# Enigmatisms/AdaPT

Measured on AMD Instinct MI355X. Metric: Msamples/s (W*H*spp/s), unidirectional MIS path tracing, higher is better.
Workload: dtype f32

## Files before the change

### adapt_amd/csrc/rng.hpp

```cpp
#pragma once
#include "vec.hpp"
#include <stdint.h>

struct Philox {
    uint32_t key0, key1, ctr0;
    uint32_t draw;
    uint32_t blk;
    uint32_t nblk;
    uint32_t c[4], n[4];
};

APT_HD void philox4x32_10(uint32_t c0, uint32_t c1, uint32_t c2, uint32_t c3, uint32_t k0, uint32_t k1, uint32_t out[4]) {
#if defined(__HIP_DEVICE_COMPILE__)
    asm volatile("" : "+v"(k0));
#endif
#pragma unroll
    for (int r = 0; r < 10; r++) {
        uint64_t p0 = (uint64_t)0xD2511F53u * c0;
        uint64_t p1 = (uint64_t)0xCD9E8D57u * c2;
        uint32_t n0 = (uint32_t)(p1 >> 32) ^ c1 ^ k0;
        uint32_t n1 = (uint32_t)p1;
        uint32_t n2 = (uint32_t)(p0 >> 32) ^ c3 ^ k1;
        uint32_t n3 = (uint32_t)p0;
        c0 = n0; c1 = n1; c2 = n2; c3 = n3;
        k0 += 0x9E3779B9u; k1 += 0xBB67AE85u;
    }
    out[0] = c0; out[1] = c1; out[2] = c2; out[3] = c3;
}

APT_HD void rng_init(Philox& r, uint32_t pixel, uint32_t seed, uint32_t sample, uint32_t draw) {
    r.key0 = pixel; r.key1 = seed; r.ctr0 = sample; r.draw = draw; r.blk = 0xffffffffu; r.nblk = 0xffffffffu;
    r.c[0] = r.c[1] = r.c[2] = r.c[3] = 0u;
    r.n[0] = r.n[1] = r.n[2] = r.n[3] = 0u;
}
APT_HD uint32_t rng_u32(Philox& r) {
    const uint32_t d = r.draw++;
    const uint32_t b = d >> 2;
    const bool step = b != r.blk;
    if (step && b != r.nblk) { philox4x32_10(r.ctr0, b, 0u, 0u, r.key0, r.key1, r.n); r.nblk = b; }
    if (step) { r.c[0] = r.n[0]; r.c[1] = r.n[1]; r.c[2] = r.n[2]; r.c[3] = r.n[3]; r.blk = b; r.nblk = 0xffffffffu; }
    const uint32_t w = d & 3u, c0 = r.c[0], c1 = r.c[1], c2 = r.c[2], c3 = r.c[3];
    return (w == 0u) ? c0 : ((w == 1u) ? c1 : ((w == 2u) ? c2 : c3));
}
APT_HD void rng_open(Philox& r) {
    const uint32_t b = r.draw >> 2;
    philox4x32_10(r.ctr0, b, 0u, 0u, r.key0, r.key1, r.c); r.blk = b;
    philox4x32_10(r.ctr0, b + 1u, 0u, 0u, r.key0, r.key1, r.n); r.nblk = b + 1u;
}
APT_HD float rng_float(Philox& r) { return (float)(rng_u32(r) >> 8) * (1.0f / 16777216.0f); }
APT_HD int32_t rng_int(Philox& r) { return (int32_t)rng_u32(r); }
APT_HD int pymod(int a, int n) { int m = a % n; return (m < 0) ? m + n : m; }
```

### adapt_amd/csrc/shade_stage.hpp

```cpp
#pragma once
#include "stages.hpp"

APT_D float ti_fmod(float a, float b) { float q = floorf(a / b); return a - b * q; }
APT_D f3 mix3(f3 a, f3 b, float t) { return a * (1.0f - t) + b * t; }
APT_D f3 texture_query(const DevScene& sc, int map, int obj, float u, float v) {
    const int* ti_ = sc.tex_i + 15 * obj + 5 * map; const float* tf = sc.tex_f + 6 * obj + 2 * map;
    const float w = (float)ti_[3], h = (float)ti_[4];
    const float scaled_u = ti_fmod((u * tf[0]) * w, w - 1.f), scaled_v = ti_fmod((v * tf[1]) * h, h - 1.f);
    float floor_u = floorf(scaled_u), floor_v = floorf(scaled_v);
    const float ratio_u = scaled_u - floor_u, ratio_v = scaled_v - floor_v;
    floor_u = floor_u + (float)ti_[1]; floor_v = floor_v + (float)ti_[2];
    const int fu = (int)floor_u, fv = (int)floor_v;
    const float* img = sc.atlas[map]; const int W = sc.atlas_w[map];
    const float* r0 = img + ((size_t)fv * W + fu) * 3; const float* r1 = r0 + (size_t)W * 3;
    const f3 q_ff = mk3(r0[0], r0[1], r0[2]), q_cf = mk3(r0[3], r0[4], r0[5]), q_fc = mk3(r1[0], r1[1], r1[2]), q_cc = mk3(r1[3], r1[4], r1[5]);
    return mix3(mix3(q_ff, q_cf, ratio_u), mix3(q_fc, q_cc, ratio_u), ratio_v);
}
APT_D bool get_uv_item(const DevScene& sc, int map, int obj, int prim, float bu, float bv, f3& out) {
    if (sc.atlas[map] == nullptr || !(sc.tex_i[15 * obj + 5 * map] > -255)) return false;
    const float* uv = sc.uvs + 6 * prim;
    const float w0 = 1.f - bu - bv;
    const float gu = (uv[2] * bu + uv[4] * bv) + uv[0] * w0, gv = (uv[3] * bu + uv[5] * bv) + uv[1] * w0;
    out = texture_query(sc, map, obj, gu, gv);
    return true;
}

APT_D void build_hit_rec(const DevScene& sc, float4 ra, float4 rb, int prim, float t, float u, float v, f3 o, f3 d, Hit& it, int& hit_light, f3& k_d, bool with_vn = true);
APT_D void build_hit(const DevScene& sc, int prim, float t, float u, float v, f3 o, f3 d, Hit& it, int& hit_light, f3& k_d) {
    build_hit_rec(sc, sc.prim_shade[2 * prim], sc.prim_shade[2 * prim + 1], prim, t, u, v, o, d, it, hit_light, k_d);
}
APT_D void build_hit_rec(const DevScene& sc, float4 ra, float4 rb, int prim, float t, float u, float v, f3 o, f3 d, Hit& it, int& hit_light, f3& k_d, bool with_vn) {
    const int code = __float_as_int(ra.w);
    it.prim_id = prim; it.min_depth = t;
    it.obj_id = (code < 0) ? ~code : code;
    hit_light = __float_as_int(rb.x);
    k_d = mk3(rb.y, rb.z, rb.w);
    if (code < 0) {
        it.n_g = normalize((o + d * t) - mk3(ra.x, ra.y, ra.z));
        it.n_s = it.n_g;
    } else {
        it.n_g = mk3(ra.x, ra.y, ra.z);
        if (with_vn && sc.has_vn) {
            const float4 v0 = sc.vnormals[3 * prim], v1 = sc.vnormals[3 * prim + 1], v2 = sc.vnormals[3 * prim + 2];
            it.n_s = (mk3(v0.x, v0.y, v0.z) * (1.f - u - v) + mk3(v1.x, v1.y, v1.z) * u) + mk3(v2.x, v2.y, v2.z) * v;
        } else it.n_s = it.n_g;
    }
}
APT_D void build_hit(const DevScene& sc, int prim, float t, float u, float v, f3 o, f3 d, Hit& it) {
    int light; f3 kd; build_hit(sc, prim, t, u, v, o, d, it, light, kd);
}

#if APT_FAST
APT_D void fix_prologue(const DevScene& sc, const Params& p, const Queues& q, Counters* cnt, int cur, int sq, int bounce) {
    const uint32_t epoch = (uint32_t)bounce + 1u;
    const int ncls = q.tr_ncls;
    uint32_t* n_def_p = &cnt->n_tr[bounce % 3][ncls][sq * CNT_PAD]; uint32_t* n_sh_p = &cnt->n_fix_sh[cur ^ 1][sq * CNT_PAD];
    const uint32_t n_def = __hip_atomic_load(n_def_p, __ATOMIC_RELAXED, __HIP_MEMORY_SCOPE_AGENT), n_sh = min(__hip_atomic_load(n_sh_p, __ATOMIC_RELAXED, __HIP_MEMORY_SCOPE_AGENT), q.sh_subcap);
    __builtin_amdgcn_fence(__ATOMIC_ACQUIRE, "workgroup");
    uint32_t old = __hip_atomic_load(&cnt->fix_claim[sq * CNT_PAD], __ATOMIC_RELAXED, __HIP_MEMORY_SCOPE_AGENT);
    if (old < epoch) {
        if ((n_def | n_sh) == 0u) return;
        if (lane_id() == 0) old = atomicMax(&cnt->fix_claim[sq * CNT_PAD], epoch);
        old = (uint32_t)__builtin_amdgcn_readlane((int)old, 0);
    }
    if (old >= epoch) {
        while (__hip_atomic_load(&cnt->fix_done[sq * CNT_PAD], __ATOMIC_ACQUIRE, __HIP_MEMORY_SCOPE_AGENT) < epoch) __builtin_amdgcn_s_sleep(16);
        return;
    }
    const uint32_t qbase = (uint32_t)sq * p.subcap, sh_qbase = (uint32_t)sq * q.sh_subcap;
    const bool need_uv = sc.has_vn || sc.tex_i != nullptr;
    for (uint32_t base = 0; base < n_def; base += 64u) {
        const uint32_t li = base + lane_id(); const bool valid = li < n_def;
        const uint32_t lj = valid ? li : n_def - 1u;
        const uint32_t io = (q.tr_stage_top ? qbase + p.subcap - n_def + lj : (uint32_t)ncls * p.cap + qbase + lj) << 4;
        const float4 ra = ldq(q.tr[cur][0], io), rb = ldq(q.tr[cur][1], io), rc = ldq(q.tr[cur][2], io), rd = ldq(q.tr[cur][3], io);
        const f3 o = mk3(ra.x, ra.y, ra.z), d = mk3(rb.x, rb.y, rb.z);
        HitRec r0, r1; r0.t = r1.t = 1e7f; r0.prim = r1.prim = -1; r0.u = r0.v = r1.u = r1.v = 0.f;
        int c0, c1;
        flat_closest2(sc.flat, sc.sweep, sc.prim_class, o, d, o, d, r0, r1, c0, c1);
        if (valid && r0.prim >= 0) {
            const int oc = ncls > 1 ? c0 : 0;
            const uint32_t pos = atomicAdd(&cnt->n_tr[bounce % 3][oc][sq * CNT_PAD], 1u);
            const uint32_t slot = (uint32_t)oc * p.cap + qbase + pos, so = slot << 4;
            stq(q.tr[cur][0], so, make_float4(ra.x, ra.y, ra.z, r0.t));
            stq(q.tr[cur][1], so, make_float4(rb.x, rb.y, rb.z, __uint_as_float((__float_as_uint(rb.w) & ~0xffu) | (uint32_t)r0.prim)));
            stq(q.tr[cur][2], so, rc); stq(q.tr[cur][3], so, rd);
            if (need_uv) { float2 uv_; uv_.x = r0.u; uv_.y = r0.v; stq(q.tr_uv[cur], slot << 3, uv_); }
        } else if (valid && !(rd.x == 0.f && rd.y == 0.f && rd.z == 0.f)) {
            const uint32_t id = __float_as_uint(rc.w), lp_ = id & ((1u << p.pix_bits) - 1u), s_ = id >> p.pix_bits;
            add_radiance(q.L, p.cap, (s_ * (uint32_t)p.npix + lp_) << 2, mk3(rd.x, rd.y, rd.z), true);
        }
    }
    uint32_t t_lit = 0;
    for (uint32_t base = 0; base < n_sh; base += 64u) {
        const uint32_t li = base + lane_id(); const bool valid = li < n_sh;
        const uint32_t io = (sh_qbase + (valid ? li : n_sh - 1u)) << 2;
        const f3 o = ld3q(q.sh_o, q.sh_cap, io), d = ld3q(q.sh_d, q.sh_cap, io), c = ld3q(q.sh_c, q.sh_cap, io);
        const float dist = ldq(q.sh_tmax, io); const uint32_t slot = ldq(q.sh_id, io);
        bool occ, occ_b;
        const float lim = (dist > 0.0f) ? dist - 1e-4f : 1e7f;
        flat_any2(sc.flat, sc.sweep, o, d, o, d, lim, lim, occ, occ_b);
        const bool weird = !(isfinite(c.x) && isfinite(c.y) && isfinite(c.z));
        const bool add = valid && (!occ || weird);
        for (unsigned long long m = __ballot(add); m != 0ull; m &= m - 1ull) {
            if ((int)lane_id() == __ffsll((long long)m) - 1) add_radiance(q.L, p.cap, slot, occ ? c * 0.f : c, true);
        }
        t_lit += (valid && !occ) ? 1u : 0u;
    }
    flush_stat(t_lit, &cnt->stats[sq][ST_LIT]);
    if (lane_id() == 0) __hip_atomic_store(n_sh_p, 0u, __ATOMIC_RELAXED, __HIP_MEMORY_SCOPE_AGENT);
    __threadfence();
    if (lane_id() == 0) __hip_atomic_store(&cnt->fix_done[sq * CNT_PAD], epoch, __ATOMIC_RELEASE, __HIP_MEMORY_SCOPE_AGENT);
}
#endif
#ifndef APT_ARGS_RELOAD
#define APT_ARGS_RELOAD 1
#endif
struct ShadeArgs3 { DevScene sc; Params p; Queues q; };
typedef const __attribute__((address_space(4))) ShadeArgs3* args3_ptr;
APT_D args3_ptr kernel_args3() { return (args3_ptr)__builtin_amdgcn_kernarg_segment_ptr(); }
APT_D const ShadeArgs3* args_fresh(args3_ptr a) {
#if APT_ARGS_RELOAD
    asm volatile("" : "+s"(a));
#endif
    return (const ShadeArgs3*)a;
}
#if APT_ARGS_RELOAD
#define APT_ARGS_PHASE() (A_ = args_fresh(A0))
#else
#define APT_ARGS_PHASE() ((void)0)
#endif
struct Vertex {
    f3 o, d, thr, hit_point; uint32_t id, l_off, draw0; float emission_weight;
    Hit it; int hit_light; DevBxdf bx;
};
APT_D void vertex_reset(Vertex& vx) {
    vx.o = splat3(0.f); vx.d = mk3(0.f, 0.f, 1.f); vx.thr = splat3(0.f); vx.hit_point = splat3(0.f); vx.id = 0; vx.l_off = 0; vx.draw0 = 0; vx.emission_weight = 1.0f;
    vx.it.obj_id = -1; vx.it.prim_id = -1; vx.it.n_s = vx.it.n_g = mk3(1.f, 0.f, 0.f); vx.it.min_depth = 0.f; vx.hit_light = -1;
    vx.bx.type = 1; vx.bx.is_delta = 0; vx.bx.is_bsdf = 0; vx.bx.k_d = vx.bx.k_s = vx.bx.k_g = vx.bx.mean = splat3(0.f); vx.bx.ior = 1.f;
}
template <int BM, int SM, int TEX>
APT_D bool open_vertex(const ShadeArgs3* A_, Vertex& vx, Philox& rng, int prim, f3 rec_kd, uint32_t meta, float ray_pdf, float2 uv, int bounce) {
    const bool was_spec = (meta >> 24) & 1u;
    if (BM == 0x002) vx.bx.k_d = rec_kd;
    else vx.bx = ld_bxdf_lane((A_->sc).bxdf + vx.it.obj_id);
    if (TEX && (A_->sc).tex_i != nullptr) {
        f3 tx;
        if (bounce == 0) {
            if (get_uv_item((A_->sc), 1, vx.it.obj_id, prim, uv.x, uv.y, tx)) { m33 R; rotation_between(mk3(0.f, 1.f, 0.f), vx.it.n_g, R); vx.it.n_s = mul(R, tx); }
            if (get_uv_item((A_->sc), 2, vx.it.obj_id, prim, uv.x, uv.y, tx)) vx.it.n_s = delocalize(vx.it.n_s, tx);
        }
        if (get_uv_item((A_->sc), 0, vx.it.obj_id, prim, uv.x, uv.y, tx)) vx.bx.k_d = tx;
    }
    const uint32_t lp = vx.id & ((1u << (A_->p).pix_bits) - 1u), s = vx.id >> (A_->p).pix_bits;
    vx.l_off = (s * (uint32_t)(A_->p).npix + lp) << 2;
    vx.draw0 = meta & 0xffffu;
    rng_init(rng, ((A_->p).world == 1) ? lp : ldq((A_->p).pix_key, lp << 2), (A_->p).seed, (uint32_t)((A_->p).cnt_base + (int)s + 1), vx.draw0);
    if (bounce > 0 && (A_->p).use_mis) {
        float e_pdf = 0.0f;
        if (vx.hit_light >= 0 && vx.bx.is_delta == 0 && !was_spec) e_pdf = emitter_solid_angle_pdf((A_->sc).src[vx.hit_light], vx.it, vx.d);
        vx.emission_weight = balance(ray_pdf, e_pdf);
    }
    if (!(SM & 2)) rng_open(rng);
    if ((A_->p).use_rr) {
        float mx = max3(vx.thr);
        if (mx < (A_->p).rr_threshold && bounce >= (A_->p).rr_bounce_th) {
            if (rng_float(rng) > mx) return false;
            vx.thr = vx.thr * srcp(mx + 1e-7f);
        }
    } else if (max3(vx.thr) < 1e-4f) return false;
    return true;
}
struct LightSample { bool want, sampled, poisoned; f3 dir, contrib; float dist, mis_w; int src; };
template <int BM, int SM, bool LANE_SRC>
APT_D LightSample sample_light(const ShadeArgs3* A_, Vertex& vx, Philox& rng, const EmitterGeom& geom, const DevSrc src_only, bool active, bool& break_flag) {
    LightSample ls; ls.want = ls.sampled = ls.poisoned = false; ls.dir = ls.contrib = splat3(0.f); ls.dist = 0.f; ls.mis_w = 1.0f; ls.src = 0;
    if (!active || break_flag) return ls;
    const int ns = (A_->sc).n_sources;
    int sidx = rng_int(rng);
    sidx = (ns == 1) ? 0 : pymod(sidx, ns);
    float emitter_pdf = (A_->p).inv_ns;
    if (vx.hit_light >= 0) {
        if (ns <= 1) { break_flag = true; return ls; }
        sidx = rng_int(rng);
        sidx = (ns == 2) ? 0 : pymod(sidx, ns - 1);
        if (sidx >= vx.hit_light) sidx += 1;
        emitter_pdf = (A_->p).inv_ns1;
    }
    DevSrc src = src_only;
    if (ns != 1) src = LANE_SRC ? ld_src_lane((A_->sc).src + sidx) : (A_->sc).src[sidx];
    ls.src = sidx;
    f3 shadow_int; float direct_pdf;
    const f3 to_emitter = emitter_sample_hit<SM>(src, geom, vx.hit_point, rng, shadow_int, direct_pdf) - vx.hit_point;
    ls.dist = fnorm(to_emitter);
    ls.dir = fdiv3(to_emitter, ls.dist);
    ls.sampled = true;
    const f3 direct_spec = surface_eval<BM>(vx.bx, vx.it, vx.d, ls.dir, (A_->sc).world_ior, (A_->p).two_sides);
    if ((A_->p).use_mis && !(src.bool_bits & 0x01)) ls.mis_w = balance(emitter_pdf * direct_pdf, surface_pdf<BM>(vx.bx, vx.it, ls.dir, vx.d, (A_->sc).world_ior, (A_->p).two_sides));
    if (isnan(ls.mis_w)) { ls.poisoned = true; return ls; }
    f3 c = (direct_spec * shadow_int) * ls.mis_w;
    if (ns != 1) c = fdiv3(c, emitter_pdf);
    ls.contrib = (c * (A_->p).inv_S) * vx.thr;
    ls.want = !(ls.contrib.x == 0.f && ls.contrib.y == 0.f && ls.contrib.z == 0.f);
    return ls;
}
template <int BM, int SM, typename Gather>
APT_D f3 emit_and_scatter(const ShadeArgs3* A_, Vertex& vx, Philox& rng, float& new_pdf, bool& is_spec, Gather&& gather) {
    if ((SM & 2) && vx.hit_light >= 0) {
        const f3 emit_int = emitter_eval_le((A_->sc).src[vx.hit_light], vx.hit_point - vx.o, vx.it.n_s);
        if (!(emit_int.x == 0.f && emit_int.y == 0.f && emit_int.z == 0.f)) gather((emit_int * vx.emission_weight) * vx.thr);
    }
    f3 spec;
    const f3 new_d = surface_sample<BM>(vx.bx, vx.it, vx.d, (A_->sc).world_ior, (A_->p).two_sides, rng, spec, new_pdf, is_spec);
    vx.thr = vx.thr * fdiv3(spec, new_pdf);
    return new_d;
}
APT_D void shadow_store(const Queues& q, uint32_t so, f3 o, f3 dir, float dist, f3 contrib) {
    st3q(q.sh_o, q.sh_cap, so, o); st3q(q.sh_d, q.sh_cap, so, dir); stq(q.sh_tmax, so, dist); st3q(q.sh_c, q.sh_cap, so, contrib);
}
struct ShadeTally { uint32_t shade, shadow, poison; };
APT_D void tally_flush(const ShadeTally& t, const uint32_t* s_draws, Counters* cnt, int sq) {
    flush_uniform(t.shade, &cnt->stats[sq][ST_SHADE]);
    flush_uniform(t.shadow, &cnt->stats[sq][ST_SHADOW]);
    if (lane_id() == 0 && s_draws[threadIdx.x >> 6]) atomicAdd(&cnt->stats[sq][ST_DRAWS], (unsigned long long)s_draws[threadIdx.x >> 6]);
    flush_uniform(t.poison, &cnt->stats[sq][ST_POISON]);
}
#if APT_FAST
template <int BM, int SM, int TEX, bool CAM = false>
APT_D void shade_traced(args3_ptr A0, Counters* cnt, int cur_, int bounce_, const unsigned long long* strips = nullptr) {
    const ShadeArgs3* A_ = args_fresh(A0);
    const int cur = CAM ? 0 : cur_, bounce = CAM ? 0 : bounce_;
    const int nxt = cur ^ 1;
    const SubLoop sl = sub_loop((A_->p).nq);
    const uint32_t qbase = (uint32_t)sl.q * (A_->p).subcap, sh_qbase = (uint32_t)sl.q * (A_->q).sh_subcap;
    uint32_t* next_counter = &cnt->n_tr[(bounce + 1) % 3][0][sl.q * CNT_PAD];
    if (sl.first == 0 && threadIdx.x == 0) {
        cnt->n_tr[(bounce + 2) % 3][0][sl.q * CNT_PAD] = 0;
        cnt->n_tr[(bounce + 2) % 3][(A_->q).tr_ncls][sl.q * CNT_PAD] = 0;
    }
    const EmitterGeom geom = {(A_->sc).precom, (A_->sc).normals, (A_->sc).obj_info};
    __shared__ uint32_t s_draws[BLOCK / 64];
    if (lane_id() == 0) s_draws[threadIdx.x >> 6] = 0;
    ShadeTally tl = {0u, 0u, 0u};
    uint32_t t_traced = 0, t_lit = 0, t_extend = 0, t_samples = 0;
#ifdef APT_NEAR_STATS
    uint32_t t_near = 0;
#endif
    constexpr bool PFP = TEX == 0 && !CAM;
    static_assert(APT_FLAT_MAX_PRIMS < (int)TR_NO_PRIM, "the packed record keeps the hit primitive in 8 bits");
    const float4* trA = (A_->q).tr[cur][0]; const float4* trB = (A_->q).tr[cur][1]; const float4* trC = (A_->q).tr[cur][2]; const float4* trD = (A_->q).tr[cur][3];
    uint32_t n, cam_total = 0;
    if constexpr (CAM) {
        cam_total = (uint32_t)(A_->p).npix * (uint32_t)(A_->p).spp_batch;
        const uint32_t n_waves = (cam_total + 63u) / 64u, nq_ = (uint32_t)(A_->p).nq;
        n = n_waves > (uint32_t)sl.q ? ((n_waves - (uint32_t)sl.q + nq_ - 1u) / nq_) * 64u : 0u;
    } else {
        fix_prologue((A_->sc), (A_->p), (A_->q), cnt, cur, sl.q, bounce);
        n = __hip_atomic_load(&cnt->n_tr[bounce % 3][0][sl.q * CNT_PAD], __ATOMIC_RELAXED, __HIP_MEMORY_SCOPE_AGENT);
    }
    uint32_t pf_pm = 0;
    auto prefetch_prim = [&](uint32_t b) { pf_pm = ldq(reinterpret_cast<const uint32_t*>(trB), ((qbase + min(b + threadIdx.x, n - 1u)) << 4) + 12u); };
    if (PFP && n > 0) prefetch_prim(sl.first);
    for (uint32_t base = sl.first; base < n; base += sl.stride) {
        APT_ARGS_PHASE();
        const uint32_t pos = base + threadIdx.x, idx = qbase + pos;
        bool alive = pos < n;
        const uint32_t cu_pm = pf_pm;
        float4 cu_ra = make_float4(0.f, 0.f, 0.f, 0.f), cu_rb = cu_ra;
        if (PFP) { const int rp = max(tr_prim(cu_pm), 0); cu_ra = (A_->sc).prim_shade[2 * rp]; cu_rb = (A_->sc).prim_shade[2 * rp + 1]; prefetch_prim(base + sl.stride); }
        Vertex vx; vertex_reset(vx);
        Philox rng; rng_init(rng, 0u, 0u, 0u, 0u);
        f3 Lc = splat3(0.f);
        bool entry = alive;
        float ray_pdf = 1.f;
        if constexpr (CAM) {
            const uint32_t w = (uint32_t)__builtin_amdgcn_readfirstlane((int)(pos >> 6)) * (uint32_t)(A_->p).nq + (uint32_t)sl.q;
            const uint32_t id_ = w * 64u + lane_id();
            const bool valid = alive && id_ < cam_total;
            f3 dir = mk3(0.f, 0.f, 1.f);
            uint32_t draws = 0;
            if (valid) {
                const uint32_t lp = id_ % (uint32_t)(A_->p).npix, s = id_ / (uint32_t)(A_->p).npix;
                int i, j; local_to_global((A_->p), lp, i, j);
                for (int pl = 0; pl < (A_->p).l_planes; pl++) stL((A_->q).L, (A_->p).cap, (id_ << 2) | (uint32_t)pl, splat3(0.f));
                dir = camera_ray_dir((A_->p), i, j, s, draws);
                vx.id = (s << (A_->p).pix_bits) | lp;
            }
            if (draws) atomicAdd(&s_draws[threadIdx.x >> 6], draws);
            const f3 cam_o = mk3((A_->p).cam_t[0], (A_->p).cam_t[1], (A_->p).cam_t[2]);
            float c_t = 0.f; int c_run = -1, c_idx = -1;
            if (__any(valid)) c_idx = flat_closest1<true>((A_->sc).flat, cam_o, dir, 1e7f, c_t, c_run, camera_strip_mask((A_->p), strips, w));
            const bool c_defer = valid && (c_run >= 0 || flat_needs_cull((A_->sc).flat, dir));
            HitRec hr; hr.t = 1e7f; hr.prim = -1; hr.u = hr.v = 0.f;
            int hit_cls = 0;
            if (valid && !c_defer && c_idx >= 0) flat_resolve((A_->sc).flat, c_idx, c_t, cam_o, dir, hr, hit_cls);
            { const uint32_t nv = wave_count(valid); t_samples += nv; t_extend += nv; }
            if (__any(c_defer)) {
                const int ncls = (A_->q).tr_ncls;
                const uint32_t dpos = wave_append(c_defer, &cnt->n_tr[0][ncls][sl.q * CNT_PAD]);
                if (c_defer) {
                    const uint32_t slot = (A_->q).tr_stage_top ? qbase + (A_->p).subcap - 1u - dpos : (uint32_t)ncls * (A_->p).cap + qbase + dpos, so = slot << 4;
                    stq((A_->q).tr[0][0], so, make_float4(cam_o.x, cam_o.y, cam_o.z, hr.t));
                    stq((A_->q).tr[0][1], so, make_float4(dir.x, dir.y, dir.z, __uint_as_float(tr_pack(hr.prim, draws, false))));
                    stq((A_->q).tr[0][2], so, make_float4(1.f, 1.f, 1.f, __uint_as_float(vx.id)));
                    stq((A_->q).tr[0][3], so, make_float4(0.f, 0.f, 0.f, 1.f));
                    if ((A_->sc).has_vn || (A_->sc).tex_i != nullptr) { float2 uv_; uv_.x = hr.u; uv_.y = hr.v; stq((A_->q).tr_uv[0], slot << 3, uv_); }
                }
            }
            entry = valid && !c_defer;
            alive = entry && hr.prim >= 0;
            if (alive) {
                vx.o = cam_o; vx.d = dir; vx.thr = splat3(1.f);
                f3 rec_kd; float2 uv; uv.x = hr.u; uv.y = hr.v;
                build_hit((A_->sc), hr.prim, hr.t, uv.x, uv.y, vx.o, vx.d, vx.it, vx.hit_light, rec_kd);
                alive = open_vertex<BM, SM, TEX>(A_, vx, rng, hr.prim, rec_kd, tr_meta(tr_pack(hr.prim, draws, false), 0u), ray_pdf, uv, 0);
            }
        }
        if (!CAM && alive && bounce > 0) { const float4 dd = ldq(trD, idx << 4); Lc = mk3(dd.x, dd.y, dd.z); if (SM & 2) ray_pdf = dd.w; }
        if (!CAM && alive) {
            const float4 a = ldq(trA, idx << 4), b_ = ldq(trB, idx << 4), c = ldq(trC, idx << 4);
            vx.o = mk3(a.x, a.y, a.z); vx.d = mk3(b_.x, b_.y, b_.z); vx.thr = mk3(c.x, c.y, c.z); vx.id = __float_as_uint(c.w);
            const uint32_t pm = PFP ? cu_pm : __float_as_uint(b_.w);
            const int prim = tr_prim(pm);
            if (prim < 0) alive = false;
            else {
                f3 rec_kd; float2 uv; uv.x = uv.y = 0.f;
                if ((A_->sc).has_vn || (TEX && (A_->sc).tex_i != nullptr)) uv = ldq((A_->q).tr_uv[cur], idx << 3);
                if (PFP) build_hit_rec((A_->sc), cu_ra, cu_rb, prim, a.w, uv.x, uv.y, vx.o, vx.d, vx.it, vx.hit_light, rec_kd);
                else build_hit((A_->sc), prim, a.w, uv.x, uv.y, vx.o, vx.d, vx.it, vx.hit_light, rec_kd);
                alive = open_vertex<BM, SM, TEX>(A_, vx, rng, prim, rec_kd, tr_meta(pm, (uint32_t)bounce), ray_pdf, uv, bounce);
            }
        }
        tl.shade += wave_count(alive);
#ifdef APT_NEAR_STATS
        t_near += wave_count(alive && bounce > 0 && vx.it.min_depth < 2e-3f);
#endif
        if (alive) vx.hit_point = vx.d * vx.it.min_depth + vx.o;

        APT_ARGS_PHASE();
        bool break_flag = false;
        DevSrc src_only;
        if ((A_->sc).n_sources == 1) src_only = ld_src_uniform((A_->sc).src);
        const LightSample f = sample_light<BM, SM, false>(A_, vx, rng, geom, src_only, alive, break_flag);
        if (f.poisoned) Lc = splat3(f.mis_w);
        tl.shadow += wave_count(f.sampled); tl.poison += wave_count(f.poisoned);
        int occ_e = 0;
        if ((A_->sc).n_sources != 1) {
            const unsigned long long wm = __ballot(f.want);
            occ_e = -1;
            if (wm != 0ull) {
                const int e0 = __builtin_amdgcn_readlane(f.src, __ffsll((long long)wm) - 1);
                if (!__any(f.want && f.src != e0)) occ_e = e0;
            }
        }
        APT_ARGS_PHASE();
        bool cont = false, is_spec = false;
        f3 new_d = mk3(0.f, 1.f, 0.f);
        float new_pdf = 1.f;
        if (alive) {
            new_d = emit_and_scatter<BM, SM>(A_, vx, rng, new_pdf, is_spec, [&](f3 add) { Lc = Lc + add; });
            cont = (bounce + 1) < (A_->p).max_bounce;
        }
        if (rng.draw != vx.draw0) atomicAdd(&s_draws[threadIdx.x >> 6], rng.draw - vx.draw0);
        APT_ARGS_PHASE();
        float tr_t = 0.f; int tr_hit = -1; float tr_u = 0.f, tr_v = 0.f; int tr_q = -1;
        TrAppend tr_app; tr_app.raw = 0u; tr_app.rank = 0u;
        {
            int tr_idx = -1, tr_run = -1, hit_cls = 0;
            if (__any(cont)) tr_idx = flat_closest1((A_->sc).flat, vx.hit_point, new_d, 1e7f, tr_t, tr_run);
            const bool tr_defer = cont && (tr_run >= 0 || flat_needs_cull((A_->sc).flat, new_d));
            t_extend += wave_count(cont);
            cont = cont && (tr_idx >= 0 || tr_defer);
            if (cont && !tr_defer) { HitRec hr; flat_resolve((A_->sc).flat, tr_idx, tr_t, vx.hit_point, new_d, hr, hit_cls); tr_hit = hr.prim; tr_u = hr.u; tr_v = hr.v; }
            tr_q = !cont ? -1 : (tr_defer ? 1 : 0);
            { const Append a_ = append_issue(tr_q == 0, next_counter); tr_app.raw = a_.raw; tr_app.rank = rank_in(a_.m); }
        }
        APT_ARGS_PHASE();
        {
            const bool defer = f.want && flat_needs_cull((A_->sc).flat, f.dir);
            bool occ = false;
            if (__any(f.want && !defer)) {
                const FlatList ls = (occ_e >= 0) ? flat_occ_list((A_->sc).flat, occ_e) : flat_full_list((A_->sc).flat);
                occ = flat_any1(ls, vx.hit_point, f.dir, (f.dist > 0.0f) ? f.dist - 1e-4f : 1e7f);
            }
            if (__any(defer)) {
                const uint32_t spos = wave_append(defer, &cnt->n_fix_sh[cur][sl.q * CNT_PAD]);
                if (defer && spos < (A_->q).sh_subcap) { const uint32_t so = (sh_qbase + spos) << 2; shadow_store((A_->q), so, vx.hit_point, f.dir, f.dist, f.contrib); stq((A_->q).sh_id, so, vx.l_off); }
            }
            const bool traced = f.want && !defer;
            if (traced) {
                const bool weird = !(isfinite(f.contrib.x) && isfinite(f.contrib.y) && isfinite(f.contrib.z));
                if (!occ || weird) Lc = Lc + (occ ? f.contrib * 0.f : f.contrib);
            }
            t_traced += wave_count(f.want); t_lit += wave_count(traced && !occ);
        }
        uint32_t npos = (uint32_t)__builtin_amdgcn_readlane((int)tr_app.raw, 0) + tr_app.rank;
        if (__any(tr_q == 1)) { const uint32_t dpos = wave_append(tr_q == 1, next_counter + APT_MAX_NQ * CNT_PAD); if (tr_q == 1) npos = dpos; }
        if (cont) {
            const uint32_t slot = (tr_q == 1) ? qbase + (A_->p).subcap - 1u - npos : qbase + npos, so = slot << 4;
            stq((A_->q).tr[nxt][0], so, make_float4(vx.hit_point.x, vx.hit_point.y, vx.hit_point.z, tr_t));
            stq((A_->q).tr[nxt][1], so, make_float4(new_d.x, new_d.y, new_d.z, __uint_as_float(tr_pack(tr_hit, rng.draw, is_spec))));
            stq((A_->q).tr[nxt][2], so, make_float4(vx.thr.x, vx.thr.y, vx.thr.z, __uint_as_float(vx.id)));
            stq((A_->q).tr[nxt][3], so, make_float4(Lc.x, Lc.y, Lc.z, new_pdf));
            if ((A_->sc).has_vn || (A_->sc).tex_i != nullptr) { float2 uv_; uv_.x = tr_u; uv_.y = tr_v; stq((A_->q).tr_uv[nxt], slot << 3, uv_); }
        }
        if (!cont && entry && !(Lc.x == 0.f && Lc.y == 0.f && Lc.z == 0.f)) {
            const uint32_t lp_ = vx.id & ((1u << (A_->p).pix_bits) - 1u), s_ = vx.id >> (A_->p).pix_bits;
            add_radiance((A_->q).L, (A_->p).cap, (s_ * (uint32_t)(A_->p).npix + lp_) << 2, Lc, true);
        }
    }
    flush_uniform(t_traced, &cnt->stats[sl.q][ST_SHADOW_TRACED]); flush_uniform(t_lit, &cnt->stats[sl.q][ST_LIT]);
    flush_uniform(t_extend, &cnt->stats[sl.q][ST_EXTEND]);
    if (CAM) flush_uniform(t_samples, &cnt->stats[sl.q][ST_SAMPLES]);
    tally_flush(tl, s_draws, cnt, sl.q);
#ifdef APT_NEAR_STATS
    flush_uniform(t_near, &cnt->stats[sl.q][14]);
#endif
}
#endif
template <int BM, int SM, int TEX, bool CQ, bool TR = false>
APT_D void shade_staged(args3_ptr A0, Counters* cnt, const ShadeIn& in, int cur, int bounce, TransQ tq = TransQ{}) {
    const ShadeArgs3* A_ = args_fresh(A0);
    const int nxt = cur ^ 1;
    const SubLoop sl = sub_loop((A_->p).nq);
    const uint32_t n = in.counts[sl.q * CNT_PAD];
    const uint32_t qbase = (uint32_t)sl.q * (A_->p).subcap, sh_qbase = (uint32_t)sl.q * (A_->q).sh_subcap;
    uint32_t* next_counter = &cnt->n_active[nxt][sl.q * CNT_PAD];
    uint32_t* shadow_counter = &cnt->n_shadow[sl.q * CNT_PAD];
    const EmitterGeom geom = {(A_->sc).precom, (A_->sc).normals, (A_->sc).obj_info};
    __shared__ uint32_t s_draws[BLOCK / 64];
    if (lane_id() == 0) s_draws[threadIdx.x >> 6] = 0;
    ShadeTally tl = {0u, 0u, 0u};
#ifdef APT_NEAR_STATS
    uint32_t t_near = 0;
#endif
    constexpr bool PFP = TEX == 0;
    const uint32_t in_base = CQ ? (uint32_t)in.cls * (A_->p).cap + qbase : qbase;
    const float4* cqA = CQ ? (A_->q).cq[0] : nullptr; const float4* cqB = CQ ? (A_->q).cq[1] : nullptr; const float4* cqC = CQ ? (A_->q).cq[2] : nullptr; const float4* cqD = CQ ? (A_->q).cq[3] : nullptr;
    int pf_prim = -1;
    auto prefetch_prim = [&](uint32_t b) {
        const uint32_t ps = in_base + min(b + threadIdx.x, n - 1u);
        pf_prim = CQ ? ldq(reinterpret_cast<const int*>(cqB), (ps << 4) + 12u) : ldq(in.prim, ps << 2);
    };
    if (PFP && n > 0) prefetch_prim(sl.first);
    for (uint32_t base = sl.first; base < n; base += sl.stride) {
        APT_ARGS_PHASE();
        const uint32_t pos = base + threadIdx.x, idx = in_base + pos;
        bool alive = pos < n;
        const int cu_prim = pf_prim;
        float4 cu_ra = make_float4(0.f, 0.f, 0.f, 0.f), cu_rb = cu_ra;
        if (PFP) { const int rp = max(cu_prim, 0); cu_ra = (A_->sc).prim_shade[2 * rp]; cu_rb = (A_->sc).prim_shade[2 * rp + 1]; prefetch_prim(base + sl.stride); }
        Vertex vx; vertex_reset(vx);
        Philox rng; rng_init(rng, 0u, 0u, 0u, 0u);
        if (alive) {
            const uint32_t io = idx << 2;
            const int prim = PFP ? cu_prim : (CQ ? ldq(reinterpret_cast<const int*>(cqB), (idx << 4) + 12u) : ldq(in.prim, io));
            if (prim < 0) alive = false;
            else {
                uint32_t meta; float t_in, ray_pdf = 1.f; float2 uv; uv.x = uv.y = 0.f;
                if (CQ) {
                    const float4 a = ldq(cqA, idx << 4), b_ = ldq(cqB, idx << 4), c = ldq(cqC, idx << 4), dd = ldq(cqD, idx << 4);
                    vx.o = mk3(a.x, a.y, a.z); t_in = a.w; vx.d = mk3(b_.x, b_.y, b_.z); vx.thr = mk3(c.x, c.y, c.z); vx.id = __float_as_uint(c.w);
                    meta = __float_as_uint(dd.x); if (SM & 2) ray_pdf = dd.y; uv.x = dd.z; uv.y = dd.w;
                } else {
                    vx.o = ld3q(in.ray_o, (A_->p).cap, io); vx.d = ld3q(in.ray_d, (A_->p).cap, io); vx.thr = ld3q(in.thr, (A_->p).cap, io);
                    vx.id = ldq(in.id, io); meta = ldq(in.meta, io); t_in = ldq(in.t, io);
                    if (SM & 2) ray_pdf = ldq(in.pdf, io);
                    if ((A_->sc).has_vn || (TEX && (A_->sc).tex_i != nullptr)) { uv.x = ldq(in.u, io); uv.y = ldq(in.v, io); }
                }
                f3 rec_kd;
                if (PFP) build_hit_rec((A_->sc), cu_ra, cu_rb, prim, t_in, uv.x, uv.y, vx.o, vx.d, vx.it, vx.hit_light, rec_kd);
                else build_hit((A_->sc), prim, t_in, uv.x, uv.y, vx.o, vx.d, vx.it, vx.hit_light, rec_kd);
                alive = open_vertex<BM, SM, TEX>(A_, vx, rng, prim, rec_kd, meta, ray_pdf, uv, bounce);
            }
        }
        tl.shade += wave_count(alive);
#ifdef APT_NEAR_STATS
        t_near += wave_count(alive && bounce > 0 && vx.it.min_depth < 2e-3f);
#endif
        if (alive) vx.hit_point = vx.d * vx.it.min_depth + vx.o;
        float t_vx = 0.f;
        if constexpr (TR) if (alive) {
            const float ior = (dot(vx.it.n_g, vx.d) < 0.f) ? (A_->sc).world_ior : (A_->sc).med[vx.it.obj_id].ior;
            t_vx = ((bounce == 0) ? 0.f : tq.t_path[vx.l_off >> 2]) + vx.it.min_depth * ior;
        }

        APT_ARGS_PHASE();
        bool break_flag = false;
        DevSrc src_only;
        if ((A_->sc).n_sources == 1) src_only = ld_src_uniform((A_->sc).src);
        uint32_t vbase = 0;
        if ((A_->p).nee_vm) vbase = wave_append(alive, shadow_counter);
        for (int s = 0; s < (A_->p).S; s++) {
            const LightSample ls = sample_light<BM, SM, CQ>(A_, vx, rng, geom, src_only, alive, break_flag);
            if (ls.poisoned) stL((A_->q).L, (A_->p).cap, vx.l_off, splat3(ls.mis_w));
            tl.shadow += wave_count(ls.sampled); tl.poison += wave_count(ls.poisoned);
            if ((A_->p).nee_vm) {
                const uint32_t so = (sh_qbase + (uint32_t)s * (A_->p).subcap + vbase) << 2;
                if (ls.want) { st3q((A_->q).sh_d, (A_->q).sh_cap, so, ls.dir); stq((A_->q).sh_tmax, so, ls.dist); st3q((A_->q).sh_c, (A_->q).sh_cap, so, ls.contrib); }
                else if (alive) stq((A_->q).sh_tmax, so, -1.0f);
                if (alive && s == 0) { stq((A_->q).sh_id, so, vx.l_off); st3q((A_->q).sh_o, (A_->q).sh_cap, so, vx.hit_point); }
            } else {
                const uint32_t spos = wave_append(ls.want, shadow_counter);
                if (ls.want && spos < (A_->q).sh_subcap) {
                    const uint32_t so = (sh_qbase + spos) << 2;
                    shadow_store((A_->q), so, vx.hit_point, ls.dir, ls.dist, ls.contrib);
                    stq((A_->q).sh_id, so, vx.l_off | (((A_->p).l_planes > 1) ? (uint32_t)s : 0u));
                    if constexpr (TR) tq.t_light[(size_t)(((A_->p).l_planes > 1) ? s : 0) * (A_->p).cap + (vx.l_off >> 2)] = t_vx + ls.dist * (A_->sc).world_ior;
                }
            }
        }
        APT_ARGS_PHASE();
        bool cont = false, is_spec = false;
        f3 new_d = mk3(0.f, 1.f, 0.f);
        float new_pdf = 1.f;
        if (alive) {
            if constexpr (TR) new_d = emit_and_scatter<BM, SM>(A_, vx, rng, new_pdf, is_spec, [&](f3 add) { tq.emit[vx.l_off >> 2] = make_float4(add.x, add.y, add.z, t_vx); });
            else new_d = emit_and_scatter<BM, SM>(A_, vx, rng, new_pdf, is_spec, [&](f3 add) { add_radiance((A_->q).L, (A_->p).cap, vx.l_off, add, true); });
            cont = (bounce + 1) < (A_->p).max_bounce;
            if constexpr (TR) if (cont) tq.t_path[vx.l_off >> 2] = t_vx;
        }
        if (rng.draw != vx.draw0) atomicAdd(&s_draws[threadIdx.x >> 6], rng.draw - vx.draw0);
        APT_ARGS_PHASE();
        const uint32_t npos = wave_append(cont, next_counter);
        if (cont) {
            const uint32_t so = (qbase + npos) << 2;
            st3q((A_->q).ray_o[nxt], (A_->p).cap, so, vx.hit_point);
            st3q((A_->q).ray_d[nxt], (A_->p).cap, so, new_d);
            st3q((A_->q).thr[nxt], (A_->p).cap, so, vx.thr);
            stq((A_->q).id[nxt], so, vx.id);
            stq((A_->q).meta[nxt], so, pack_meta(rng.draw, (uint32_t)(bounce + 1), is_spec));
            if (SM & 2) stq((A_->q).pdf[nxt], so, new_pdf);
        }
    }
    tally_flush(tl, s_draws, cnt, sl.q);
#ifdef APT_NEAR_STATS
    flush_uniform(t_near, &cnt->stats[sl.q][14]);
#endif
}
template <int BM, int SM, int TEX = 0>
__global__ void __launch_bounds__(BLOCK) k_shade(DevScene sc, Params p, Queues q, Counters* cnt, ShadeIn in, int cur, int bounce) {
    shade_staged<BM, SM, TEX, false>(kernel_args3(), cnt, in, cur, bounce);
}
template <int BM, int SM, int TEX = 0>
__global__ void __launch_bounds__(BLOCK) k_shade_tr(DevScene sc, Params p, Queues q, Counters* cnt, ShadeIn in, int cur, int bounce, TransQ tq) {
    shade_staged<BM, SM, TEX, false, true>(kernel_args3(), cnt, in, cur, bounce, tq);
}
#if APT_FAST
template <int BM, int SM, int TEX = 0>
__global__ void __launch_bounds__(BLOCK) k_shade_traced(DevScene sc, Params p, Queues q, Counters* cnt, int cur, int bounce) {
    shade_traced<BM, SM, TEX>(kernel_args3(), cnt, cur, bounce);
}
#ifndef APT_TRACED_WAVES
#define APT_TRACED_WAVES 7
#endif
template <int BM, int SM>
__global__ void __launch_bounds__(BLOCK) __attribute__((amdgpu_waves_per_eu(APT_TRACED_WAVES, APT_TRACED_WAVES))) k_shade_traced_lean(DevScene sc, Params p, Queues q, Counters* cnt, int cur, int bounce) {
    shade_traced<BM, SM, 0>(kernel_args3(), cnt, cur, bounce);
}
template <int BM, int SM, int TEX = 0>
__global__ void __launch_bounds__(BLOCK) k_shade_traced_cam(DevScene sc, Params p, Queues q, Counters* cnt, const unsigned long long* strips) {
    shade_traced<BM, SM, TEX, true>(kernel_args3(), cnt, 0, 0, strips);
}
#ifndef APT_TRACED_CAM_WAVES
#define APT_TRACED_CAM_WAVES 7
#endif
template <int BM, int SM>
__global__ void __launch_bounds__(BLOCK) __attribute__((amdgpu_waves_per_eu(APT_TRACED_CAM_WAVES, APT_TRACED_CAM_WAVES))) k_shade_traced_lean_cam(DevScene sc, Params p, Queues q, Counters* cnt, const unsigned long long* strips) {
    shade_traced<BM, SM, 0, true>(kernel_args3(), cnt, 0, 0, strips);
}
#endif

#define APT_GROUP_SLOTS 6
struct GroupIn { const uint32_t* counts[APT_GROUP_SLOTS]; int cls[APT_GROUP_SLOTS]; };
template <int SM, int WAVES, int B0, int B1, int B2, int B3, int B4 = 0, int B5 = 0>
__global__ void __launch_bounds__(BLOCK, WAVES) k_shade_group(DevScene sc, Params p, Queues q, Counters* cnt, GroupIn g, int cur, int bounce) {
    ShadeIn in = {nullptr, nullptr, nullptr, nullptr, nullptr, nullptr, nullptr, nullptr, nullptr, nullptr, nullptr, 0};
    if constexpr (B0 != 0) if (g.cls[0] >= 0) { in.counts = g.counts[0]; in.cls = g.cls[0]; shade_staged<B0, SM, 0, true>(kernel_args3(), cnt, in, cur, bounce); }
    if constexpr (B1 != 0) if (g.cls[1] >= 0) { in.counts = g.counts[1]; in.cls = g.cls[1]; shade_staged<B1, SM, 0, true>(kernel_args3(), cnt, in, cur, bounce); }
    if constexpr (B2 != 0) if (g.cls[2] >= 0) { in.counts = g.counts[2]; in.cls = g.cls[2]; shade_staged<B2, SM, 0, true>(kernel_args3(), cnt, in, cur, bounce); }
    if constexpr (B4 != 0) if (g.cls[4] >= 0) { in.counts = g.counts[4]; in.cls = g.cls[4]; shade_staged<B4, SM, 0, true>(kernel_args3(), cnt, in, cur, bounce); }
    if constexpr (B5 != 0) if (g.cls[5] >= 0) { in.counts = g.counts[5]; in.cls = g.cls[5]; shade_staged<B5, SM, 0, true>(kernel_args3(), cnt, in, cur, bounce); }
    if constexpr (B3 != 0) if (g.cls[3] >= 0) { in.counts = g.counts[3]; in.cls = g.cls[3]; shade_staged<B3, SM, 0, true>(kernel_args3(), cnt, in, cur, bounce); }
}
template <int SM, int B0, int B1, int B2, int B3, int B4 = 0, int B5 = 0>
__global__ void __launch_bounds__(BLOCK) k_shade_group_tr(DevScene sc, Params p, Queues q, Counters* cnt, GroupIn g, int cur, int bounce, TransQ tq) {
    ShadeIn in = {nullptr, nullptr, nullptr, nullptr, nullptr, nullptr, nullptr, nullptr, nullptr, nullptr, nullptr, 0};
    if constexpr (B0 != 0) if (g.cls[0] >= 0) { in.counts = g.counts[0]; in.cls = g.cls[0]; shade_staged<B0, SM, 0, true, true>(kernel_args3(), cnt, in, cur, bounce, tq); }
    if constexpr (B1 != 0) if (g.cls[1] >= 0) { in.counts = g.counts[1]; in.cls = g.cls[1]; shade_staged<B1, SM, 0, true, true>(kernel_args3(), cnt, in, cur, bounce, tq); }
    if constexpr (B2 != 0) if (g.cls[2] >= 0) { in.counts = g.counts[2]; in.cls = g.cls[2]; shade_staged<B2, SM, 0, true, true>(kernel_args3(), cnt, in, cur, bounce, tq); }
    if constexpr (B4 != 0) if (g.cls[4] >= 0) { in.counts = g.counts[4]; in.cls = g.cls[4]; shade_staged<B4, SM, 0, true, true>(kernel_args3(), cnt, in, cur, bounce, tq); }
    if constexpr (B5 != 0) if (g.cls[5] >= 0) { in.counts = g.counts[5]; in.cls = g.cls[5]; shade_staged<B5, SM, 0, true, true>(kernel_args3(), cnt, in, cur, bounce, tq); }
    if constexpr (B3 != 0) if (g.cls[3] >= 0) { in.counts = g.counts[3]; in.cls = g.cls[3]; shade_staged<B3, SM, 0, true, true>(kernel_args3(), cnt, in, cur, bounce, tq); }
}
```

Baseline: 5994.

## Interleave paired Philox blocks and make shade front-end branch-free

rng_open now computes both Philox blocks in one interleaved loop, which exposes instruction-level parallelism across the two independent multiply chains. The shade loop drops the divergent `if (alive)` wrappers. It clamps the queue index and primitive id so every lane runs the camera-ray, hit-build and vertex-open code uniformly, and it masks the results afterwards with `shaded`. Dead initialisations are replaced by opaque asm 'unread' values, and the constants in the store path are materialised from a hidden zero, both to cut register and instruction pressure. In exchange, inactive lanes do redundant loads and arithmetic, and the stats bookkeeping changes to account for the lanes that were previously skipped.

```diff
diff --git a/adapt_amd/csrc/rng.hpp b/adapt_amd/csrc/rng.hpp
--- a/adapt_amd/csrc/rng.hpp
+++ b/adapt_amd/csrc/rng.hpp
@@ -42,10 +42,27 @@
     const uint32_t w = d & 3u, c0 = r.c[0], c1 = r.c[1], c2 = r.c[2], c3 = r.c[3];
     return (w == 0u) ? c0 : ((w == 1u) ? c1 : ((w == 2u) ? c2 : c3));
 }
+APT_HD void philox4x32_10_pair(uint32_t c0, uint32_t b, uint32_t k0, uint32_t k1, uint32_t out_b[4], uint32_t out_b1[4]) {
+#if defined(__HIP_DEVICE_COMPILE__)
+    asm volatile("" : "+v"(k0));
+#endif
+    uint32_t x0 = c0, x1 = b, x2 = 0u, x3 = 0u, y0 = c0, y1 = b + 1u, y2 = 0u, y3 = 0u;
+#pragma unroll
+    for (int r = 0; r < 10; r++) {
+        const uint64_t px0 = (uint64_t)0xD2511F53u * x0, px1 = (uint64_t)0xCD9E8D57u * x2;
+        const uint64_t py0 = (uint64_t)0xD2511F53u * y0, py1 = (uint64_t)0xCD9E8D57u * y2;
+        const uint32_t nx0 = (uint32_t)(px1 >> 32) ^ x1 ^ k0, nx2 = (uint32_t)(px0 >> 32) ^ x3 ^ k1;
+        const uint32_t ny0 = (uint32_t)(py1 >> 32) ^ y1 ^ k0, ny2 = (uint32_t)(py0 >> 32) ^ y3 ^ k1;
+        x0 = nx0; x1 = (uint32_t)px1; x2 = nx2; x3 = (uint32_t)px0;
+        y0 = ny0; y1 = (uint32_t)py1; y2 = ny2; y3 = (uint32_t)py0;
+        k0 += 0x9E3779B9u; k1 += 0xBB67AE85u;
+    }
+    out_b[0] = x0; out_b[1] = x1; out_b[2] = x2; out_b[3] = x3;
+    out_b1[0] = y0; out_b1[1] = y1; out_b1[2] = y2; out_b1[3] = y3;
+}
 APT_HD void rng_open(Philox& r) {
     const uint32_t b = r.draw >> 2;
-    philox4x32_10(r.ctr0, b, 0u, 0u, r.key0, r.key1, r.c); r.blk = b;
-    philox4x32_10(r.ctr0, b + 1u, 0u, 0u, r.key0, r.key1, r.n); r.nblk = b + 1u;
+    philox4x32_10_pair(r.ctr0, b, r.key0, r.key1, r.c, r.n); r.blk = b; r.nblk = b + 1u;
 }
 APT_HD float rng_float(Philox& r) { return (float)(rng_u32(r) >> 8) * (1.0f / 16777216.0f); }
 APT_HD int32_t rng_int(Philox& r) { return (int32_t)rng_u32(r); }
diff --git a/adapt_amd/csrc/shade_stage.hpp b/adapt_amd/csrc/shade_stage.hpp
--- a/adapt_amd/csrc/shade_stage.hpp
+++ b/adapt_amd/csrc/shade_stage.hpp
@@ -130,6 +130,8 @@
 #else
 #define APT_ARGS_PHASE() ((void)0)
 #endif
+template <typename T> APT_D T unread() { T x; asm volatile("" : "=v"(x)); return x; }
+APT_D f3 unread3() { return mk3(unread<float>(), unread<float>(), unread<float>()); }
 struct Vertex {
     f3 o, d, thr, hit_point; uint32_t id, l_off, draw0; float emission_weight;
     Hit it; int hit_light; DevBxdf bx;
@@ -172,9 +174,11 @@
     return true;
 }
 struct LightSample { bool want, sampled, poisoned; f3 dir, contrib; float dist, mis_w; int src; };
-template <int BM, int SM, bool LANE_SRC>
+template <int BM, int SM, bool LANE_SRC, bool BARE = false>
 APT_D LightSample sample_light(const ShadeArgs3* A_, Vertex& vx, Philox& rng, const EmitterGeom& geom, const DevSrc src_only, bool active, bool& break_flag) {
-    LightSample ls; ls.want = ls.sampled = ls.poisoned = false; ls.dir = ls.contrib = splat3(0.f); ls.dist = 0.f; ls.mis_w = 1.0f; ls.src = 0;
+    LightSample ls; ls.want = ls.sampled = ls.poisoned = false;
+    if (BARE) { ls.dir = unread3(); ls.contrib = unread3(); ls.dist = unread<float>(); ls.mis_w = unread<float>(); ls.src = unread<int>(); }
+    else { ls.dir = ls.contrib = splat3(0.f); ls.dist = 0.f; ls.mis_w = 1.0f; ls.src = 0; }
     if (!active || break_flag) return ls;
     const int ns = (A_->sc).n_sources;
     int sidx = rng_int(rng);
@@ -195,6 +199,7 @@
     ls.dist = fnorm(to_emitter);
     ls.dir = fdiv3(to_emitter, ls.dist);
     ls.sampled = true;
+    if (BARE) ls.mis_w = 1.0f;
     const f3 direct_spec = surface_eval<BM>(vx.bx, vx.it, vx.d, ls.dir, (A_->sc).world_ior, (A_->p).two_sides);
     if ((A_->p).use_mis && !(src.bool_bits & 0x01)) ls.mis_w = balance(emitter_pdf * direct_pdf, surface_pdf<BM>(vx.bx, vx.it, ls.dir, vx.d, (A_->sc).world_ior, (A_->p).two_sides));
     if (isnan(ls.mis_w)) { ls.poisoned = true; return ls; }
@@ -241,6 +246,7 @@
     const EmitterGeom geom = {(A_->sc).precom, (A_->sc).normals, (A_->sc).obj_info};
     __shared__ uint32_t s_draws[BLOCK / 64];
     if (lane_id() == 0) s_draws[threadIdx.x >> 6] = 0;
+    auto draws_slot = [&]() -> uint32_t* { uint32_t t = threadIdx.x; asm volatile("" : "+v"(t)); return &s_draws[t >> 6]; };
     ShadeTally tl = {0u, 0u, 0u};
     uint32_t t_traced = 0, t_lit = 0, t_extend = 0, t_samples = 0;
 #ifdef APT_NEAR_STATS
@@ -263,30 +269,29 @@
     if (PFP && n > 0) prefetch_prim(sl.first);
     for (uint32_t base = sl.first; base < n; base += sl.stride) {
         APT_ARGS_PHASE();
-        const uint32_t pos = base + threadIdx.x, idx = qbase + pos;
-        bool alive = pos < n;
+        const uint32_t pos = base + threadIdx.x, idx = qbase + min(pos, n - 1u);
+        const bool entry_q = pos < n;
         const uint32_t cu_pm = pf_pm;
         float4 cu_ra = make_float4(0.f, 0.f, 0.f, 0.f), cu_rb = cu_ra;
         if (PFP) { const int rp = max(tr_prim(cu_pm), 0); cu_ra = (A_->sc).prim_shade[2 * rp]; cu_rb = (A_->sc).prim_shade[2 * rp + 1]; prefetch_prim(base + sl.stride); }
-        Vertex vx; vertex_reset(vx);
-        Philox rng; rng_init(rng, 0u, 0u, 0u, 0u);
+        Vertex vx; Philox rng;
+        vx.emission_weight = 1.0f;
+        if (BM == 0x002) { vx.bx.type = 1; vx.bx.is_delta = 0; vx.bx.is_bsdf = 0; vx.bx.k_s = vx.bx.k_g = vx.bx.mean = splat3(0.f); vx.bx.ior = 1.f; }
         f3 Lc = splat3(0.f);
-        bool entry = alive;
+        bool entry, shaded, alive;
         float ray_pdf = 1.f;
         if constexpr (CAM) {
             const uint32_t w = (uint32_t)__builtin_amdgcn_readfirstlane((int)(pos >> 6)) * (uint32_t)(A_->p).nq + (uint32_t)sl.q;
-            const uint32_t id_ = w * 64u + lane_id();
-            const bool valid = alive && id_ < cam_total;
-            f3 dir = mk3(0.f, 0.f, 1.f);
+            const uint32_t id_live = w * 64u + lane_id();
+            const bool valid = id_live < cam_total;
+            const uint32_t id_ = valid ? id_live : 0u;
+            const uint32_t lp = id_ % (uint32_t)(A_->p).npix, s = id_ / (uint32_t)(A_->p).npix;
+            int i, j; local_to_global((A_->p), lp, i, j);
+            if (valid) for (int pl = 0; pl < (A_->p).l_planes; pl++) stL((A_->q).L, (A_->p).cap, (id_ << 2) | (uint32_t)pl, splat3(0.f));
             uint32_t draws = 0;
-            if (valid) {
-                const uint32_t lp = id_ % (uint32_t)(A_->p).npix, s = id_ / (uint32_t)(A_->p).npix;
-                int i, j; local_to_global((A_->p), lp, i, j);
-                for (int pl = 0; pl < (A_->p).l_planes; pl++) stL((A_->q).L, (A_->p).cap, (id_ << 2) | (uint32_t)pl, splat3(0.f));
-                dir = camera_ray_dir((A_->p), i, j, s, draws);
-                vx.id = (s << (A_->p).pix_bits) | lp;
-            }
-            if (draws) atomicAdd(&s_draws[threadIdx.x >> 6], draws);
+            const f3 dir = camera_ray_dir((A_->p), i, j, s, draws);
+            vx.id = (s << (A_->p).pix_bits) | lp;
+            if (valid && draws) atomicAdd(draws_slot(), draws);
             const f3 cam_o = mk3((A_->p).cam_t[0], (A_->p).cam_t[1], (A_->p).cam_t[2]);
             float c_t = 0.f; int c_run = -1, c_idx = -1;
             if (__any(valid)) c_idx = flat_closest1<true>((A_->sc).flat, cam_o, dir, 1e7f, c_t, c_run, camera_strip_mask((A_->p), strips, w));
@@ -294,54 +299,53 @@
             HitRec hr; hr.t = 1e7f; hr.prim = -1; hr.u = hr.v = 0.f;
             int hit_cls = 0;
             if (valid && !c_defer && c_idx >= 0) flat_resolve((A_->sc).flat, c_idx, c_t, cam_o, dir, hr, hit_cls);
-            { const uint32_t nv = wave_count(valid); t_samples += nv; t_extend += nv; }
+            t_samples += min(64u, cam_total - min(cam_total, w * 64u));
             if (__any(c_defer)) {
                 const int ncls = (A_->q).tr_ncls;
                 const uint32_t dpos = wave_append(c_defer, &cnt->n_tr[0][ncls][sl.q * CNT_PAD]);
                 if (c_defer) {
                     const uint32_t slot = (A_->q).tr_stage_top ? qbase + (A_->p).subcap - 1u - dpos : (uint32_t)ncls * (A_->p).cap + qbase + dpos, so = slot << 4;
+                    uint32_t zero_bits = 0u; asm volatile("" : "+v"(zero_bits));
+                    const float zero = __uint_as_float(zero_bits), one = __uint_as_float(zero_bits | 0x3f800000u);
                     stq((A_->q).tr[0][0], so, make_float4(cam_o.x, cam_o.y, cam_o.z, hr.t));
                     stq((A_->q).tr[0][1], so, make_float4(dir.x, dir.y, dir.z, __uint_as_float(tr_pack(hr.prim, draws, false))));
-                    stq((A_->q).tr[0][2], so, make_float4(1.f, 1.f, 1.f, __uint_as_float(vx.id)));
-                    stq((A_->q).tr[0][3], so, make_float4(0.f, 0.f, 0.f, 1.f));
+                    stq((A_->q).tr[0][2], so, make_float4(one, one, one, __uint_as_float(vx.id)));
+                    stq((A_->q).tr[0][3], so, make_float4(zero, zero, zero, one));
                     if ((A_->sc).has_vn || (A_->sc).tex_i != nullptr) { float2 uv_; uv_.x = hr.u; uv_.y = hr.v; stq((A_->q).tr_uv[0], slot << 3, uv_); }
                 }
             }
             entry = valid && !c_defer;
-            alive = entry && hr.prim >= 0;
-            if (alive) {
-                vx.o = cam_o; vx.d = dir; vx.thr = splat3(1.f);
-                f3 rec_kd; float2 uv; uv.x = hr.u; uv.y = hr.v;
-                build_hit((A_->sc), hr.prim, hr.t, uv.x, uv.y, vx.o, vx.d, vx.it, vx.hit_light, rec_kd);
-                alive = open_vertex<BM, SM, TEX>(A_, vx, rng, hr.prim, rec_kd, tr_meta(tr_pack(hr.prim, draws, false), 0u), ray_pdf, uv, 0);
-            }
-        }
-        if (!CAM && alive && bounce > 0) { const float4 dd = ldq(trD, idx << 4); Lc = mk3(dd.x, dd.y, dd.z); if (SM & 2) ray_pdf = dd.w; }
-        if (!CAM && alive) {
+            shaded = entry && hr.prim >= 0;
+            const int prim = max(hr.prim, 0);
+            vx.o = cam_o; vx.d = dir; vx.thr = splat3(1.f);
+            f3 rec_kd; float2 uv; uv.x = hr.u; uv.y = hr.v;
+            build_hit((A_->sc), prim, hr.t, uv.x, uv.y, vx.o, vx.d, vx.it, vx.hit_light, rec_kd);
+            alive = open_vertex<BM, SM, TEX>(A_, vx, rng, prim, rec_kd, tr_meta(tr_pack(prim, draws, false), 0u), ray_pdf, uv, 0) && shaded;
+        } else {
+            entry = entry_q;
+            if (bounce > 0) { const float4 dd = ldq(trD, idx << 4); Lc = mk3(dd.x, dd.y, dd.z); if (SM & 2) ray_pdf = dd.w; }
             const float4 a = ldq(trA, idx << 4), b_ = ldq(trB, idx << 4), c = ldq(trC, idx << 4);
             vx.o = mk3(a.x, a.y, a.z); vx.d = mk3(b_.x, b_.y, b_.z); vx.thr = mk3(c.x, c.y, c.z); vx.id = __float_as_uint(c.w);
             const uint32_t pm = PFP ? cu_pm : __float_as_uint(b_.w);
-            const int prim = tr_prim(pm);
-            if (prim < 0) alive = false;
-            else {
-                f3 rec_kd; float2 uv; uv.x = uv.y = 0.f;
-                if ((A_->sc).has_vn || (TEX && (A_->sc).tex_i != nullptr)) uv = ldq((A_->q).tr_uv[cur], idx << 3);
-                if (PFP) build_hit_rec((A_->sc), cu_ra, cu_rb, prim, a.w, uv.x, uv.y, vx.o, vx.d, vx.it, vx.hit_light, rec_kd);
-                else build_hit((A_->sc), prim, a.w, uv.x, uv.y, vx.o, vx.d, vx.it, vx.hit_light, rec_kd);
-                alive = open_vertex<BM, SM, TEX>(A_, vx, rng, prim, rec_kd, tr_meta(pm, (uint32_t)bounce), ray_pdf, uv, bounce);
-            }
+            shaded = entry && tr_prim(pm) >= 0;
+            const int prim = max(tr_prim(pm), 0);
+            f3 rec_kd; float2 uv; uv.x = uv.y = 0.f;
+            if ((A_->sc).has_vn || (TEX && (A_->sc).tex_i != nullptr)) uv = ldq((A_->q).tr_uv[cur], idx << 3);
+            if (PFP) build_hit_rec((A_->sc), cu_ra, cu_rb, prim, a.w, uv.x, uv.y, vx.o, vx.d, vx.it, vx.hit_light, rec_kd);
+            else build_hit((A_->sc), prim, a.w, uv.x, uv.y, vx.o, vx.d, vx.it, vx.hit_light, rec_kd);
+            alive = open_vertex<BM, SM, TEX>(A_, vx, rng, prim, rec_kd, tr_meta(pm, (uint32_t)bounce), ray_pdf, uv, bounce) && shaded;
         }
         tl.shade += wave_count(alive);
 #ifdef APT_NEAR_STATS
         t_near += wave_count(alive && bounce > 0 && vx.it.min_depth < 2e-3f);
 #endif
-        if (alive) vx.hit_point = vx.d * vx.it.min_depth + vx.o;
+        vx.hit_point = vx.d * vx.it.min_depth + vx.o;
 
         APT_ARGS_PHASE();
         bool break_flag = false;
         DevSrc src_only;
         if ((A_->sc).n_sources == 1) src_only = ld_src_uniform((A_->sc).src);
-        const LightSample f = sample_light<BM, SM, false>(A_, vx, rng, geom, src_only, alive, break_flag);
+        const LightSample f = sample_light<BM, SM, false, true>(A_, vx, rng, geom, src_only, alive, break_flag);
         if (f.poisoned) Lc = splat3(f.mis_w);
         tl.shadow += wave_count(f.sampled); tl.poison += wave_count(f.poisoned);
         int occ_e = 0;
@@ -355,13 +359,13 @@
         }
         APT_ARGS_PHASE();
         bool cont = false, is_spec = false;
-        f3 new_d = mk3(0.f, 1.f, 0.f);
-        float new_pdf = 1.f;
+        f3 new_d = unread3();
+        float new_pdf = unread<float>();
         if (alive) {
             new_d = emit_and_scatter<BM, SM>(A_, vx, rng, new_pdf, is_spec, [&](f3 add) { Lc = Lc + add; });
             cont = (bounce + 1) < (A_->p).max_bounce;
         }
-        if (rng.draw != vx.draw0) atomicAdd(&s_draws[threadIdx.x >> 6], rng.draw - vx.draw0);
+        if (shaded && rng.draw != vx.draw0) atomicAdd(draws_slot(), rng.draw - vx.draw0);
         APT_ARGS_PHASE();
         float tr_t = 0.f; int tr_hit = -1; float tr_u = 0.f, tr_v = 0.f; int tr_q = -1;
         TrAppend tr_app; tr_app.raw = 0u; tr_app.rank = 0u;
@@ -404,13 +408,13 @@
             stq((A_->q).tr[nxt][3], so, make_float4(Lc.x, Lc.y, Lc.z, new_pdf));
             if ((A_->sc).has_vn || (A_->sc).tex_i != nullptr) { float2 uv_; uv_.x = tr_u; uv_.y = tr_v; stq((A_->q).tr_uv[nxt], slot << 3, uv_); }
         }
-        if (!cont && entry && !(Lc.x == 0.f && Lc.y == 0.f && Lc.z == 0.f)) {
+        if (!cont && (CAM || entry) && !(Lc.x == 0.f && Lc.y == 0.f && Lc.z == 0.f)) {
             const uint32_t lp_ = vx.id & ((1u << (A_->p).pix_bits) - 1u), s_ = vx.id >> (A_->p).pix_bits;
             add_radiance((A_->q).L, (A_->p).cap, (s_ * (uint32_t)(A_->p).npix + lp_) << 2, Lc, true);
         }
     }
     flush_uniform(t_traced, &cnt->stats[sl.q][ST_SHADOW_TRACED]); flush_uniform(t_lit, &cnt->stats[sl.q][ST_LIT]);
-    flush_uniform(t_extend, &cnt->stats[sl.q][ST_EXTEND]);
+    flush_uniform(t_extend + (CAM ? t_samples : 0u), &cnt->stats[sl.q][ST_EXTEND]);
     if (CAM) flush_uniform(t_samples, &cnt->stats[sl.q][ST_SAMPLES]);
     tally_flush(tl, s_draws, cnt, sl.q);
 #ifdef APT_NEAR_STATS
```

Result: faster. 6096, median of 6 (+1.7%).
